# Shadylukin/Neumann

Measured on AMD Instinct MI355X. Metric: queries/sec, brute-force SIMILAR TOP-K (recall@K = 1.0 vs CPU oracle), higher is better.
Workload: dtype f32

## Files before the change

### neumann_amd/csrc/nmn_scan_ring.hip

```cpp
#include <algorithm>
#include <cstdlib>

#include "nmn_internal.h"

namespace nmn {

namespace {

typedef float f4 __attribute__((ext_vector_type(4)));
typedef uint32_t u4 __attribute__((ext_vector_type(4)));

constexpr int kRingStageBytes = 64 * 128 * 4;
constexpr int kRingStages = 4;
constexpr int kRingPieces = 8;
constexpr int kRingRowPitch = 128;
constexpr uint32_t kRingTailWeight = 4;

#ifdef NMN_RING_WG_CLOCK
__device__ unsigned long long* nmn_ring_clk;
#define NMN_RING_CLK(i, v) do { if (threadIdx.x == 0) nmn_ring_clk[(uint64_t)blockIdx.x * 5u + (i)] = (v); } while (0)
#else
#define NMN_RING_CLK(i, v) do { } while (0)
#endif

template <int N>
__device__ __forceinline__ void ring_wait_vm() {
    asm volatile("s_waitcnt vmcnt(%0)" ::"n"(N) : "memory");
}

template <int METRIC, bool PROBE = false>
__global__ void __launch_bounds__(256, 1) scan_ring_kernel(ScanParams p) {
    extern __shared__ __attribute__((aligned(16))) float lds[];
    float* const nrm = lds + kRingStages * (kRingStageBytes / 4);
    uint32_t* const tpart = reinterpret_cast<uint32_t*>(nrm + 8 * 64);
    float* const qlds = nrm + 8 * 64 + 8;
    const uint32_t KC = p.ld / 128u;
    constexpr bool kL2 = METRIC == NMN_METRIC_EUCLIDEAN;
    constexpr bool kCos = METRIC == NMN_METRIC_COSINE;
    const uint32_t lane = threadIdx.x & 63u;
    const uint32_t wave = __builtin_amdgcn_readfirstlane(threadIdx.x >> 6);
    const uint32_t r4 = lane >> 4, j = lane & 15u;
    const uint32_t ld = p.ld;
    const uint32_t row_bytes = ld * 4u;
    NMN_RING_CLK(0, wall_clock64());
    NMN_RING_CLK(4, __smid());
    const uint32_t tpw = p.tiles_per_wave;
    auto first_tile = [&](uint32_t b) -> uint32_t {
        const uint64_t gm = p.ring_wgs - p.ring_tail;
        const uint64_t u = b <= gm ? (uint64_t)kRingTailWeight * b : (uint64_t)kRingTailWeight * gm + (b - gm);
        return (uint32_t)(u * p.n_tiles / ((uint64_t)kRingTailWeight * gm + p.ring_tail));
    };
    uint32_t* const ticket = reinterpret_cast<uint32_t*>(qlds + ld);
    for (uint32_t round = 0;; round++) {
    uint32_t bx = blockIdx.x;
    if (p.ring_wgs) {
        if (threadIdx.x == 0) *ticket = atomicAdd(p.ring_ctr, 1u);
        __syncthreads();
        bx = __builtin_amdgcn_readfirstlane(*ticket);
        __syncthreads();
        if (bx >= p.ring_wgs) break;
    } else if (round) {
        break;
    }
    const uint32_t t0 = p.ring_wgs ? first_tile(bx) : bx * tpw;
    const uint32_t t1 = p.ring_wgs ? first_tile(bx + 1u) : min(t0 + tpw, p.n_tiles);
    if (t0 >= p.n_tiles || t1 <= t0) continue;
    const uint32_t n_stage = (t1 - t0) * KC;

    for (uint32_t c = wave; !PROBE && c * 256u < ld; c += 4u) {
        if (c * 256u + lane * 4u < ld)
            __builtin_amdgcn_global_load_lds((const __attribute__((address_space(1))) void*)(p.qpad + c * 256u + lane * 4u),
                                             (__attribute__((address_space(3))) void*)(qlds + c * 256u), 16, 0, 0);
    }
    const float qmag = PROBE ? 1.f : p.qinfo[0].qmag;

    uint32_t loff[kRingPieces];
#pragma unroll
    for (int pp = 0; pp < kRingPieces; pp++) {
        const uint32_t r = 2u * (wave * kRingPieces + (uint32_t)pp) + lane / 32u;
        loff[pp] = r * row_bytes + (((lane % 32u) ^ (r & 15u)) * 16u);
    }
    const char* const mat = reinterpret_cast<const char*>(p.corpus);
    auto stage_src = [&](uint32_t tile_, uint32_t kc_) -> const char* {
        return mat + (uint64_t)tile_ * kTileRows * row_bytes + (uint64_t)kc_ * 512u;
    };
    auto issue_stage = [&](const char* src, uint32_t lmask, uint32_t slot) __attribute__((always_inline)) {
#pragma unroll
        for (int pp = 0; pp < kRingPieces; pp++)
            __builtin_amdgcn_global_load_lds((const __attribute__((address_space(1))) void*)(src + (loff[pp] & lmask)),
                                             (__attribute__((address_space(3))) void*)(lds + slot * (kRingStageBytes / 4) +
                                                                                        (wave * kRingPieces + (uint32_t)pp) * 256u),
                                             16, 0, 2);
    };
    auto norms_dma = [&](uint32_t tile_, uint32_t rel) __attribute__((always_inline)) {
        __builtin_amdgcn_global_load_lds((const __attribute__((address_space(1))) void*)(p.norms + (uint64_t)tile_ * kTileRows + lane),
                                         (__attribute__((address_space(3))) void*)(nrm + (rel & 7u) * 64u), 4, 0, 0);
    };
#pragma unroll
    for (uint32_t s0 = 0; s0 < kRingStages; s0++) {
        if (s0 < n_stage) {
            if (!PROBE && kCos && wave == 0 && s0 % KC == 0) norms_dma(t0 + s0 / KC, s0 / KC);
            if (s0 < kRingStages - 1) issue_stage(stage_src(t0 + s0 / KC, s0 % KC), 0xFFFFFFFFu, s0 % kRingStages);
        } else if (s0 < kRingStages - 1) {
            issue_stage(mat, 0u, s0 % kRingStages);
        }
    }
    constexpr int kSub = 4;
    uint32_t off[kSub];
#pragma unroll
    for (int sub = 0; sub < kSub; sub++) {
        const uint32_t rr = (uint32_t)sub * 4u + r4;
        off[sub] = (wave * 16u + rr) * kRingRowPitch + (((j * 2u) ^ rr) * 4u);
    }

    uint32_t wmax = kKeyMasked;
    auto flush_group = [&](uint32_t g, uint32_t m) __attribute__((always_inline)) {
        if (lane != 0) return;
        if (g * tpw >= t0 && min(g * tpw + tpw, p.n_tiles) <= t1) p.wmax[g] = m;
        else atomicMax(p.wmax + g, m);
    };
    uint32_t sidx = 0;
    uint32_t nt = t0 + (kRingStages - 1) / KC, nkc = (kRingStages - 1) % KC;
    for (uint32_t tile = t0; tile < t1; tile++) {
        float acc[kSub][2];
#pragma unroll
        for (int sub = 0; sub < kSub; sub++) acc[sub][0] = acc[sub][1] = 0.f;
        for (uint32_t kc = 0; kc < KC; kc++, sidx++) {
            const float* buf = lds + (sidx % kRingStages) * (kRingStageBytes / 4);
            ring_wait_vm<(kRingStages - 2) * kRingPieces>();
            if (kc == 0) __builtin_amdgcn_s_barrier();
            asm volatile("" ::: "memory");
            if (sidx == 0) NMN_RING_CLK(1, wall_clock64());
            if (!PROBE && kc == 0 && wave == 0 && tile > t0) {
                const uint32_t* tp = tpart + ((tile - 1u - t0) & 1u) * 4u;
                const uint32_t m = max(max(tp[0], tp[1]), max(tp[2], tp[3]));
                if (lane == 0) p.tmax[tile - 1u] = m;
                wmax = max(wmax, m);
                if (tile % tpw == 0) {
                    flush_group((tile - 1u) / tpw, wmax);
                    wmax = kKeyMasked;
                }
            }
            const uint32_t ns = sidx + (kRingStages - 1);
            const bool issue = ns < n_stage;
            if (ns == n_stage) NMN_RING_CLK(2, wall_clock64());
            const char* const nsrc = issue ? stage_src(nt, nkc) : mat;
            const uint32_t lmask = issue ? 0xFFFFFFFFu : 0u;
            float* const nbuf = lds + (ns % kRingStages) * (kRingStageBytes / 4);
            f4 a[kSub][2];
            f4 q0 = {0.f, 0.f, 0.f, 0.f}, q1 = q0;
            if constexpr (!PROBE) {
#pragma unroll
                for (int sub = 0; sub < kSub; sub++) {
                    a[sub][0] = *reinterpret_cast<const f4*>(buf + off[sub]);
                    a[sub][1] = *reinterpret_cast<const f4*>(buf + (off[sub] ^ 4u));
                }
                q0 = *reinterpret_cast<const f4*>(qlds + kc * 128u + j * 8u);
                q1 = *reinterpret_cast<const f4*>(qlds + kc * 128u + j * 8u + 4u);
            }
#pragma unroll
            for (int sub = 0; sub < kSub; sub++) {
#pragma unroll
                for (int pp = sub * 2; pp < sub * 2 + 2; pp++)
                    __builtin_amdgcn_global_load_lds((const __attribute__((address_space(1))) void*)(nsrc + (loff[pp] & lmask)),
                                                     (__attribute__((address_space(3))) void*)(nbuf + (wave * kRingPieces + (uint32_t)pp) * 256u), 16, 0, 2);
                if constexpr (PROBE) continue;
                const f4 x0 = a[sub][0], x1 = a[sub][1];
                if constexpr (kL2) {
                    const f4 d0 = x0 - q0, d1 = x1 - q1;
#pragma unroll
                    for (int e = 0; e < 4; e++) {
                        acc[sub][0] = __builtin_fmaf(d0[e], d0[e], acc[sub][0]);
                        acc[sub][1] = __builtin_fmaf(d1[e], d1[e], acc[sub][1]);
                    }
                } else {
#pragma unroll
                    for (int e = 0; e < 4; e++) {
                        acc[sub][0] = __builtin_fmaf(x0[e], q0[e], acc[sub][0]);
                        acc[sub][1] = __builtin_fmaf(x1[e], q1[e], acc[sub][1]);
                    }
                }
            }
            asm volatile("s_waitcnt lgkmcnt(0)" ::: "memory");
            if (++nkc == KC) {
                nkc = 0;
                nt++;
            }
            if (!PROBE && kCos && wave == 0 && ns + 1u < n_stage && nkc == 0) norms_dma(nt, nt - t0);
        }
        if constexpr (PROBE) continue;
        float v = 0.f;
#pragma unroll
        for (int sub = 0; sub < kSub; sub++) {
            float t = acc[sub][0] + acc[sub][1];
            t += __int_as_float(__builtin_amdgcn_update_dpp(0, __float_as_int(t), 0x128, 0xF, 0xF, false));
            t += __int_as_float(__builtin_amdgcn_update_dpp(0, __float_as_int(t), 0x124, 0xF, 0xF, false));
            t += __int_as_float(__builtin_amdgcn_update_dpp(0, __float_as_int(t), 0x122, 0xF, 0xF, false));
            t += __int_as_float(__builtin_amdgcn_update_dpp(0, __float_as_int(t), 0x121, 0xF, 0xF, false));
            if ((j & 3u) == (uint32_t)sub) v = t;
        }
        const uint32_t wrow = (j & 3u) * 4u + r4;
        const uint64_t row = (uint64_t)tile * kTileRows + wave * 16u + wrow;
        const bool valid = row < p.n_rows;
        float sc;
        if constexpr (kCos) {
            const float vn = nrm[((tile - t0) & 7u) * 64u + wave * 16u + wrow];
            sc = (vn == 0.f || qmag == 0.f) ? 0.f : v / (qmag * vn);
        } else if constexpr (kL2) {
            const float dist = sqrtf(fmaxf(v, 0.f));
            sc = p.metric == kMetricNegL2 ? -dist : 1.0f / (1.0f + dist);
        } else {
            sc = v;
        }
        uint32_t key = valid ? score_to_key(sc) : kKeyMasked;
        if (j < 4u) p.scores[row] = valid ? f2u(sc) : kScoreSentinelBits;
#pragma unroll
        for (int o = 1; o < 64; o <<= 1) key = max(key, (uint32_t)__shfl_xor((int)key, o));
        if (lane == 0) tpart[((tile - t0) & 1u) * 4u + wave] = key;
        asm volatile("s_waitcnt lgkmcnt(0)" ::: "memory");
    }
    ring_wait_vm<0>();
    __builtin_amdgcn_s_barrier();
    asm volatile("" ::: "memory");
    if (!PROBE && wave == 0) {
        const uint32_t* tp = tpart + ((t1 - 1u - t0) & 1u) * 4u;
        const uint32_t m = max(max(tp[0], tp[1]), max(tp[2], tp[3]));
        wmax = max(wmax, m);
        if (lane == 0) p.tmax[t1 - 1u] = m;
        flush_group((t1 - 1u) / tpw, wmax);
    }
    }
    if (p.ring_wgs && threadIdx.x == 0 && atomicAdd(p.ring_ctr + 1, 1u) == gridDim.x - 1u) {
        p.ring_ctr[0] = 0u;
        p.ring_ctr[1] = 0u;
    }
    NMN_RING_CLK(3, wall_clock64());
}

template <int METRIC>
hipError_t launch_ring_metric(const ScanParams& p, hipStream_t s) {
    const uint32_t blocks = p.ring_wgs ? p.ring_grid : (p.n_tiles + p.tiles_per_wave - 1) / p.tiles_per_wave;
    const size_t lds = (size_t)kRingStages * kRingStageBytes + 8 * 64 * 4 + 8 * 4 + (size_t)p.ld * 4 + 16;
    auto kern = scan_ring_kernel<METRIC>;
    hipError_t e = hipFuncSetAttribute(reinterpret_cast<const void*>(kern), hipFuncAttributeMaxDynamicSharedMemorySize, (int)lds);
    if (e != hipSuccess) return e;
    hipLaunchKernelGGL(kern, dim3(blocks), dim3(256), lds, s, p);
    return hipGetLastError();
}

}

bool scan_ring_supported(uint32_t ld, uint32_t dim, int metric) {
    if (!(metric == NMN_METRIC_COSINE || metric == NMN_METRIC_DOT_PRODUCT || metric == NMN_METRIC_EUCLIDEAN || metric == kMetricNegL2)) return false;
    return dim <= ld && ld % 128u == 0 && ld >= 128u && ld <= 4096u;
}

void ring_set_grid(ScanParams& p, uint32_t* ctr) {
    struct Grid {
        uint32_t chunks, tail, wgs;
    };
    static const Grid g = []() -> Grid {
        if (getenv("NMN_NO_RING_EVEN")) return {0, 0, 0};
        int dev = 0, n = 256;
        if (hipGetDevice(&dev) != hipSuccess || hipDeviceGetAttribute(&n, hipDeviceAttributeMultiprocessorCount, dev) != hipSuccess || n <= 0) n = 256;
        auto knob = [](const char* name, long def) {
            const char* e = getenv(name);
            return std::min<long>(std::max<long>(e ? atol(e) : def, 0), 32);
        };
        const long m = std::max<long>(knob("NMN_RING_MAIN", 14), 1), t = knob("NMN_RING_TAIL", 8);
        return {(uint32_t)((m + t) * n), (uint32_t)(t * n), (uint32_t)n};
    }();
    p.ring_wgs = ctr ? g.chunks : 0u;
    p.ring_tail = g.tail;
    p.ring_grid = g.wgs;
    p.ring_ctr = ctr;
}

hipError_t launch_ring_probe(const float* corpus, uint64_t n_rows, uint32_t ld, uint32_t tiles_per_wg, uint32_t* ctr, hipStream_t s) {
    ScanParams p{};
    p.corpus = corpus;
    p.n_rows = n_rows;
    p.ld = ld;
    p.n_tiles = (uint32_t)(n_rows / kTileRows);
    p.tiles_per_wave = std::max<uint32_t>(1, tiles_per_wg);
    ring_set_grid(p, ctr);
    if (p.n_tiles == 0) return hipSuccess;
    const uint32_t blocks = p.ring_wgs ? p.ring_grid : (p.n_tiles + p.tiles_per_wave - 1) / p.tiles_per_wave;
    const size_t lds = (size_t)kRingStages * kRingStageBytes + 8 * 64 * 4 + 8 * 4 + (size_t)p.ld * 4 + 16;
    auto kern = scan_ring_kernel<NMN_METRIC_DOT_PRODUCT, true>;
    hipError_t e = hipFuncSetAttribute(reinterpret_cast<const void*>(kern), hipFuncAttributeMaxDynamicSharedMemorySize, (int)lds);
    if (e != hipSuccess) return e;
    hipLaunchKernelGGL(kern, dim3(blocks), dim3(256), lds, s, p);
    return hipGetLastError();
}

hipError_t launch_scan_ring(const ScanParams& p, hipStream_t s) {
    switch (p.metric) {
        case NMN_METRIC_COSINE: return launch_ring_metric<NMN_METRIC_COSINE>(p, s);
        case NMN_METRIC_EUCLIDEAN:
        case kMetricNegL2: return launch_ring_metric<NMN_METRIC_EUCLIDEAN>(p, s);
        default: return launch_ring_metric<NMN_METRIC_DOT_PRODUCT>(p, s);
    }
}

}
```

Baseline: 227.5.

## Hoist per-chunk setup out of ring loop and scale chunk count to corpus size

```diff
diff --git a/neumann_amd/csrc/nmn_scan_ring.hip b/neumann_amd/csrc/nmn_scan_ring.hip
--- a/neumann_amd/csrc/nmn_scan_ring.hip
+++ b/neumann_amd/csrc/nmn_scan_ring.hip
@@ -18,9 +18,15 @@
 
 #ifdef NMN_RING_WG_CLOCK
 __device__ unsigned long long* nmn_ring_clk;
+__device__ unsigned long long* nmn_ring_cclk;
+constexpr uint32_t kRingClkChunks = 64;
 #define NMN_RING_CLK(i, v) do { if (threadIdx.x == 0) nmn_ring_clk[(uint64_t)blockIdx.x * 5u + (i)] = (v); } while (0)
+#define NMN_RING_CCLK(c, i, v) do { if (threadIdx.x == 0 && (c) < kRingClkChunks) nmn_ring_cclk[((uint64_t)blockIdx.x * kRingClkChunks + (c)) * 6u + (i)] = (v); } while (0)
+#define NMN_RING_CLK_ONLY(x) x
 #else
 #define NMN_RING_CLK(i, v) do { } while (0)
+#define NMN_RING_CCLK(c, i, v) do { } while (0)
+#define NMN_RING_CLK_ONLY(x)
 #endif
 
 template <int N>
@@ -51,6 +57,47 @@
         return (uint32_t)(u * p.n_tiles / ((uint64_t)kRingTailWeight * gm + p.ring_tail));
     };
     uint32_t* const ticket = reinterpret_cast<uint32_t*>(qlds + ld);
+    const float* const qmag_lds = qlds + ld + 1u;
+    for (uint32_t c = wave; !PROBE && c * 256u < ld; c += 4u) {
+        if (c * 256u + lane * 4u < ld)
+            __builtin_amdgcn_global_load_lds((const __attribute__((address_space(1))) void*)(p.qpad + c * 256u + lane * 4u),
+                                             (__attribute__((address_space(3))) void*)(qlds + c * 256u), 16, 0, 0);
+    }
+    if (!PROBE && kCos && wave == 0 && lane == 0)
+        __builtin_amdgcn_global_load_lds((const __attribute__((address_space(1))) void*)&p.qinfo[0].qmag,
+                                         (__attribute__((address_space(3))) void*)qmag_lds, 4, 0, 0);
+
+    uint32_t loff[kRingPieces];
+#pragma unroll
+    for (int pp = 0; pp < kRingPieces; pp++) {
+        const uint32_t r = 2u * (wave * kRingPieces + (uint32_t)pp) + lane / 32u;
+        loff[pp] = r * row_bytes + (((lane % 32u) ^ (r & 15u)) * 16u);
+    }
+    const char* const mat = reinterpret_cast<const char*>(p.corpus);
+    auto stage_src = [&](uint32_t tile_, uint32_t kc_) -> const char* {
+        return mat + (uint64_t)tile_ * kTileRows * row_bytes + (uint64_t)kc_ * 512u;
+    };
+    auto issue_stage = [&](const char* src, uint32_t lmask, uint32_t slot) __attribute__((always_inline)) {
+#pragma unroll
+        for (int pp = 0; pp < kRingPieces; pp++)
+            __builtin_amdgcn_global_load_lds((const __attribute__((address_space(1))) void*)(src + (loff[pp] & lmask)),
+                                             (__attribute__((address_space(3))) void*)(lds + slot * (kRingStageBytes / 4) +
+                                                                                        (wave * kRingPieces + (uint32_t)pp) * 256u),
+                                             16, 0, 2);
+    };
+    auto norms_dma = [&](uint32_t tile_, uint32_t rel) __attribute__((always_inline)) {
+        __builtin_amdgcn_global_load_lds((const __attribute__((address_space(1))) void*)(p.norms + (uint64_t)tile_ * kTileRows + lane),
+                                         (__attribute__((address_space(3))) void*)(nrm + (rel & 7u) * 64u), 4, 0, 0);
+    };
+    constexpr int kSub = 4;
+    uint32_t off[kSub];
+#pragma unroll
+    for (int sub = 0; sub < kSub; sub++) {
+        const uint32_t rr = (uint32_t)sub * 4u + r4;
+        off[sub] = (wave * 16u + rr) * kRingRowPitch + (((j * 2u) ^ rr) * 4u);
+    }
+
+    NMN_RING_CLK_ONLY(uint32_t cidx = 0;)
     for (uint32_t round = 0;; round++) {
     uint32_t bx = blockIdx.x;
     if (p.ring_wgs) {
@@ -64,38 +111,13 @@
     }
     const uint32_t t0 = p.ring_wgs ? first_tile(bx) : bx * tpw;
     const uint32_t t1 = p.ring_wgs ? first_tile(bx + 1u) : min(t0 + tpw, p.n_tiles);
+    NMN_RING_CCLK(cidx, 0, wall_clock64());
     if (t0 >= p.n_tiles || t1 <= t0) continue;
     const uint32_t n_stage = (t1 - t0) * KC;
-
-    for (uint32_t c = wave; !PROBE && c * 256u < ld; c += 4u) {
-        if (c * 256u + lane * 4u < ld)
-            __builtin_amdgcn_global_load_lds((const __attribute__((address_space(1))) void*)(p.qpad + c * 256u + lane * 4u),
-                                             (__attribute__((address_space(3))) void*)(qlds + c * 256u), 16, 0, 0);
-    }
-    const float qmag = PROBE ? 1.f : p.qinfo[0].qmag;
-
-    uint32_t loff[kRingPieces];
-#pragma unroll
-    for (int pp = 0; pp < kRingPieces; pp++) {
-        const uint32_t r = 2u * (wave * kRingPieces + (uint32_t)pp) + lane / 32u;
-        loff[pp] = r * row_bytes + (((lane % 32u) ^ (r & 15u)) * 16u);
-    }
-    const char* const mat = reinterpret_cast<const char*>(p.corpus);
-    auto stage_src = [&](uint32_t tile_, uint32_t kc_) -> const char* {
-        return mat + (uint64_t)tile_ * kTileRows * row_bytes + (uint64_t)kc_ * 512u;
-    };
-    auto issue_stage = [&](const char* src, uint32_t lmask, uint32_t slot) __attribute__((always_inline)) {
-#pragma unroll
-        for (int pp = 0; pp < kRingPieces; pp++)
-            __builtin_amdgcn_global_load_lds((const __attribute__((address_space(1))) void*)(src + (loff[pp] & lmask)),
-                                             (__attribute__((address_space(3))) void*)(lds + slot * (kRingStageBytes / 4) +
-                                                                                        (wave * kRingPieces + (uint32_t)pp) * 256u),
-                                             16, 0, 2);
-    };
-    auto norms_dma = [&](uint32_t tile_, uint32_t rel) __attribute__((always_inline)) {
-        __builtin_amdgcn_global_load_lds((const __attribute__((address_space(1))) void*)(p.norms + (uint64_t)tile_ * kTileRows + lane),
-                                         (__attribute__((address_space(3))) void*)(nrm + (rel & 7u) * 64u), 4, 0, 0);
-    };
+    NMN_RING_CCLK(cidx, 5, n_stage);
+    NMN_RING_CCLK(cidx, 1, wall_clock64());
+    if (n_stage <= kRingStages - 1) NMN_RING_CCLK(cidx, 3, wall_clock64());
+
 #pragma unroll
     for (uint32_t s0 = 0; s0 < kRingStages; s0++) {
         if (s0 < n_stage) {
@@ -105,14 +127,6 @@
             issue_stage(mat, 0u, s0 % kRingStages);
         }
     }
-    constexpr int kSub = 4;
-    uint32_t off[kSub];
-#pragma unroll
-    for (int sub = 0; sub < kSub; sub++) {
-        const uint32_t rr = (uint32_t)sub * 4u + r4;
-        off[sub] = (wave * 16u + rr) * kRingRowPitch + (((j * 2u) ^ rr) * 4u);
-    }
-
     uint32_t wmax = kKeyMasked;
     auto flush_group = [&](uint32_t g, uint32_t m) __attribute__((always_inline)) {
         if (lane != 0) return;
@@ -131,6 +145,7 @@
             if (kc == 0) __builtin_amdgcn_s_barrier();
             asm volatile("" ::: "memory");
             if (sidx == 0) NMN_RING_CLK(1, wall_clock64());
+            if (sidx == 0) NMN_RING_CCLK(cidx, 2, wall_clock64());
             if (!PROBE && kc == 0 && wave == 0 && tile > t0) {
                 const uint32_t* tp = tpart + ((tile - 1u - t0) & 1u) * 4u;
                 const uint32_t m = max(max(tp[0], tp[1]), max(tp[2], tp[3]));
@@ -144,6 +159,7 @@
             const uint32_t ns = sidx + (kRingStages - 1);
             const bool issue = ns < n_stage;
             if (ns == n_stage) NMN_RING_CLK(2, wall_clock64());
+            if (ns + 1u == n_stage) NMN_RING_CCLK(cidx, 3, wall_clock64());
             const char* const nsrc = issue ? stage_src(nt, nkc) : mat;
             const uint32_t lmask = issue ? 0xFFFFFFFFu : 0u;
             float* const nbuf = lds + (ns % kRingStages) * (kRingStageBytes / 4);
@@ -205,6 +221,7 @@
         float sc;
         if constexpr (kCos) {
             const float vn = nrm[((tile - t0) & 7u) * 64u + wave * 16u + wrow];
+            const float qmag = *qmag_lds;
             sc = (vn == 0.f || qmag == 0.f) ? 0.f : v / (qmag * vn);
         } else if constexpr (kL2) {
             const float dist = sqrtf(fmaxf(v, 0.f));
@@ -219,6 +236,8 @@
         if (lane == 0) tpart[((tile - t0) & 1u) * 4u + wave] = key;
         asm volatile("s_waitcnt lgkmcnt(0)" ::: "memory");
     }
+    NMN_RING_CCLK(cidx, 4, wall_clock64());
+    NMN_RING_CLK_ONLY(cidx++;)
     ring_wait_vm<0>();
     __builtin_amdgcn_s_barrier();
     asm volatile("" ::: "memory");
@@ -256,11 +275,13 @@
 }
 
 void ring_set_grid(ScanParams& p, uint32_t* ctr) {
+    constexpr uint32_t kRingMinShareTiles = 2;
     struct Grid {
-        uint32_t chunks, tail, wgs;
+        uint32_t main, tail, wgs;
+        bool fixed;
     };
     static const Grid g = []() -> Grid {
-        if (getenv("NMN_NO_RING_EVEN")) return {0, 0, 0};
+        if (getenv("NMN_NO_RING_EVEN")) return {0, 0, 0, true};
         int dev = 0, n = 256;
         if (hipGetDevice(&dev) != hipSuccess || hipDeviceGetAttribute(&n, hipDeviceAttributeMultiprocessorCount, dev) != hipSuccess || n <= 0) n = 256;
         auto knob = [](const char* name, long def) {
@@ -268,10 +289,17 @@
             return std::min<long>(std::max<long>(e ? atol(e) : def, 0), 32);
         };
         const long m = std::max<long>(knob("NMN_RING_MAIN", 14), 1), t = knob("NMN_RING_TAIL", 8);
-        return {(uint32_t)((m + t) * n), (uint32_t)(t * n), (uint32_t)n};
+        return {(uint32_t)m, (uint32_t)t, (uint32_t)n, getenv("NMN_RING_MAIN") || getenv("NMN_RING_TAIL")};
     }();
-    p.ring_wgs = ctr ? g.chunks : 0u;
-    p.ring_tail = g.tail;
+    uint32_t m = g.main, t = g.tail;
+    const uint64_t shares = (uint64_t)(kRingTailWeight * m + t) * g.wgs;
+    if (!g.fixed && p.n_tiles < kRingMinShareTiles * shares) {
+        const double f = (double)p.n_tiles / (double)(kRingMinShareTiles * shares);
+        m = std::max<uint32_t>(1, (uint32_t)(m * f + 0.5));
+        t = std::max<uint32_t>(1, (uint32_t)(t * f + 0.5));
+    }
+    p.ring_wgs = ctr ? (m + t) * g.wgs : 0u;
+    p.ring_tail = t * g.wgs;
     p.ring_grid = g.wgs;
     p.ring_ctr = ctr;
 }
```

Result: no change. 227.5, median of 2 (-0.0%).
